# lxjeffffff/PagedAttention-Based-Transformer-Decoder-Inference-Framework

Hardware: AMD Instinct MI355X
Metric: decode tokens/sec at batch=64 seq_len=8192; % HBM-roofline (1/2/4/8 GPU) (higher is better)
Workload: dtype int8 GEMM (i32 acc) + fp16 KV attention (fp32 acc); 1 GPU; C3: INT8 decoder (MFMA i8 matmuls + fp16 paged attention), 24-layer/16-head/d=128, batch 64, KV context 8192, page 16; strong scaling: 64 rows over 1 GPU(s); global_batch=64, batch_per_gpu=64, seq_len=8192, page_size=16, parallelism=single GPU (no collective)

## Files before the change

pagedattention-based-transformer-decoder-inference-framework_amd/csrc/gemm_impl.hpp:

```cpp
#pragma once

#include "common.hpp"
#include "fp8.hpp"
#include "gemm.hpp"
#include "ln_wave.hpp"

namespace llm {

struct KvAppend {
  const int32_t* pos;
  const int32_t* page_table;
  const int32_t* rows;
  _Float16* k_pool;
  _Float16* v_pool;
  int num_beams, max_tiles, TS, num_pages, H, D;
  size_t page_stride;
  int fp8;
  float k_inv, v_inv;
};

struct GemmArgs {
  const uint8_t* A;
  int lda;
  int a_packed;
  const uint8_t* B;
  int M, N, K, KS;
  const float* sa;
  const float* sw;
  const float* bias;
  int act;
  float* C;
  int32_t* acc_out;
  int c_cols;
  int c_ld;
  _Float16* c16;
  KvAppend kv;
  unsigned long long* stamps;
  const float* ln_x;
  const _Float16* ln_emb;
  const int32_t* ln_tok;
  int ln_V;
  const float* ln_g;
  const float* ln_b;
  float ln_eps;
  uint8_t* act_out;
  float* sa_out;
  int partial;
  int w_keep;
  int xcd_map;
  unsigned* seam;
  int seam_n;
  int qdiag;
  int ksplit2;
};

__host__ __device__ constexpr int ln_row_stride(int K, int esize) { return K * esize + 32; }

__device__ __forceinline__ unsigned long long phase_clock() {
  unsigned long long t;
  asm volatile("s_memrealtime %0\n\ts_waitcnt lgkmcnt(0)" : "=s"(t)::"memory");
  return t;
}


template <int MT, int WAVES, int NT = 1>
constexpr int gemm_unroll() {
  return (MT >= 4 ? 2 : 4) * (WAVES == 4 ? 2 : 1) / (NT >= 4 ? 2 : 1);
}

__device__ __forceinline__ float apply_act(float y, int act) {
  if (act == LLM_ACT_RELU) return fmaxf(y, 0.f);
  if (act == LLM_ACT_GELU) return 0.5f * y * (1.f + erff(y * 0.70710678118654752f));
  return y;
}

enum class GemmKind { I8, F16 };

template <GemmKind KIND>
struct GemmTraits;
template <>
struct GemmTraits<GemmKind::I8> {
  static constexpr int KSTEP = 64, ESIZE = 1;
  using acc_t = i32x4;
  using elem_t = int32_t;
};
template <>
struct GemmTraits<GemmKind::F16> {
  static constexpr int KSTEP = 32, ESIZE = 2;
  using acc_t = f32x4;
  using elem_t = float;
};

template <GemmKind KIND, int ROWS, int WAVES>
__device__ __forceinline__ void ln_prologue(const GemmArgs& a, int m0, uint8_t* alds,
                                            float* sa_lds) {
  constexpr int ESIZE = GemmTraits<KIND>::ESIZE;
  constexpr int CPL = 8;
  const int lane = lane_id();
  const int w = wave_id_uniform();
  const int K = a.K;
  const int K4 = K >> 2;
  const int stride = ln_row_stride(K, ESIZE);
  const bool do_ln = a.ln_g != nullptr;
  LnRow<CPL> gm, bt;
  ln_wave_load(a.ln_g, K4, do_ln, gm);
  ln_wave_load(a.ln_b, K4, do_ln, bt);
  for (int r0 = w; r0 < ROWS; r0 += 2 * WAVES) {
    LnRow<CPL> x[2];
#pragma unroll
    for (int q = 0; q < 2; ++q) {
      const int r = r0 + q * WAVES;
      const int m = m0 + r;
      const bool ok = r < ROWS && m < a.M;
      if (a.ln_emb)
        ln_wave_load_f16(ok ? ln_embed_row(a.ln_emb, a.ln_tok, m, a.ln_V, K) : a.ln_emb, K4, ok,
                         x[q]);
      else
        ln_wave_load(a.ln_x + (size_t)m * K, K4, ok, x[q]);
    }
#pragma unroll
    for (int q = 0; q < 2; ++q) {
      const int r = r0 + q * WAVES;
      if (r >= ROWS) break;
      const bool mok = m0 + r < a.M;
      float am;
      if (do_ln) {
        am = ln_wave_compute(x[q], gm, bt, K, a.ln_eps);
      } else {
        am = 0.f;
#pragma unroll
        for (int j = 0; j < CPL; ++j)
#pragma unroll
          for (int e = 0; e < 4; ++e) am = fmaxf(am, fabsf(x[q].v[j][e]));
        am = ln_wave_max(am);
      }
      uint8_t* rowp = alds + (size_t)r * stride;
      if constexpr (KIND == GemmKind::I8) {
        const float scale = 127.f / (am + 1e-6f);
#pragma unroll
        for (int j = 0; j < CPL; ++j) {
          const int c = 64 * j + lane;
          if (c < K4)
            *reinterpret_cast<uint32_t*>(rowp + 4 * c) = mok ? ln_quant4(x[q].v[j], scale) : 0u;
        }
        if (lane == 0) sa_lds[r] = mok ? 1.0f / scale : 0.f;
      } else {
#pragma unroll
        for (int j = 0; j < CPL; ++j) {
          const int c = 64 * j + lane;
          if (c < K4)
            *reinterpret_cast<ln_f16x4*>(rowp + 8 * c) =
                mok ? ln_half4(x[q].v[j]) : ln_f16x4{0, 0, 0, 0};
        }
      }
    }
  }
}

__device__ __forceinline__ void seam_wait(unsigned* ctr, int n) {
  if (threadIdx.x == 0) {
    unsigned spins = 0;
    while (__hip_atomic_load(&ctr[0], __ATOMIC_RELAXED, __HIP_MEMORY_SCOPE_AGENT) < (unsigned)n) {
      __builtin_amdgcn_s_sleep(8);
      if (++spins > (1u << 21)) {
        __hip_atomic_store(&ctr[2], 1u, __ATOMIC_RELAXED, __HIP_MEMORY_SCOPE_AGENT);
        break;
      }
    }
    __builtin_amdgcn_fence(__ATOMIC_ACQUIRE, "agent");
  }
  __syncthreads();
}

template <GemmKind KIND, int MT, int NT, int WAVES, int DIAG = 0, int PRO = 0, int SEAM = 0>
__device__ __forceinline__ void gemm_tile(const GemmArgs& a, int bx, int by, int bz, int nz,
                                          int gx) {
  using Tr = GemmTraits<KIND>;
  using acc_t = typename Tr::acc_t;
  constexpr int KSTEP = Tr::KSTEP;
  constexpr int kUnroll = gemm_unroll<MT, WAVES, NT>();
  using elem_t = typename Tr::elem_t;
  using RedT = elem_t[MT * NT][4][64];
  extern __shared__ __attribute__((aligned(16))) uint8_t gemm_smem[];
  RedT* red;
  if constexpr (PRO == 0) {
    __shared__ elem_t red_static[WAVES][MT * NT][4][64];
    red = red_static;
  } else {
    red = reinterpret_cast<RedT*>(gemm_smem);
  }
  constexpr int ROWS_ = 16 * MT;
  const int a_stride = ln_row_stride(a.K, Tr::ESIZE);
  uint8_t* alds = gemm_smem;
  float* sa_lds = reinterpret_cast<float*>(gemm_smem + (size_t)ROWS_ * a_stride);

  const int lane = lane_id();
  const int w = wave_id_uniform();
  const int nt0 = bx * NT;
  const int m0 = by * 16 * MT;
  unsigned long long* stamp =
      a.stamps ? a.stamps + ((size_t)by * gx + bx) * 48 : nullptr;
  if (stamp && lane == 0) stamp[w] = phase_clock();
  const int wr = (w + bx) % WAVES;
  const int kz0 = (int)((bz * a.KS) / nz);
  const int kzn = (int)(((bz + 1) * a.KS) / nz) - kz0;
  const int ks0 = kz0 + (wr * kzn) / WAVES;
  const int ks1 = kz0 + ((wr + 1) * kzn) / WAVES;
  const int ntiles = (a.N + 15) >> 4;

  const int arow_lane = lane & 15;
  const int kgrp = lane >> 4;
  const bool apk = a.a_packed;
  const uint32_t a_bytes = apk ? (uint32_t)(((a.M + 15) / 16) * a.KS * 1024u)
                               : (uint32_t)((size_t)a.M * a.lda * Tr::ESIZE);
  const auto arsrc = __builtin_amdgcn_make_buffer_rsrc((void*)a.A, (short)0, a_bytes, 0x00020000);
  const uint32_t a_kstride = apk ? 1024u : (uint32_t)(KSTEP * Tr::ESIZE);
  const uint32_t a_kgrp_off = apk ? 0u : (uint32_t)(kgrp * (KSTEP / 4) * Tr::ESIZE);
  uint32_t a_row_off[MT];
#pragma unroll
  for (int mt = 0; mt < MT; ++mt) {
    const int row = m0 + mt * 16 + arow_lane;
    a_row_off[mt] = row >= a.M ? 0xFFFFFFF0u
                    : apk ? (uint32_t)((((m0 >> 4) + mt) * a.KS) * 1024u + lane * 16)
                          : (uint32_t)((size_t)row * a.lda * Tr::ESIZE);
  }
  const uint8_t* bbase = a.B + (size_t)nt0 * a.KS * 1024;
  const uint32_t b_bytes = (uint32_t)(min(NT, ntiles - nt0) * a.KS * 1024u);
  uint32_t b_lane_off[NT];
#pragma unroll
  for (int j = 0; j < NT; ++j) b_lane_off[j] = (uint32_t)j * a.KS * 1024u + lane * 16;
  const auto brsrc = __builtin_amdgcn_make_buffer_rsrc((void*)bbase, (short)0, b_bytes, 0x00020000);

  acc_t acc[MT][NT];
#pragma unroll
  for (int mt = 0; mt < MT; ++mt)
#pragma unroll
    for (int j = 0; j < NT; ++j) acc[mt][j] = acc_t{0, 0, 0, 0};

  struct Batch {
    u32x4 b[kUnroll][NT];
    u32x4 af[kUnroll][MT];
  };
  auto issue = [&](Batch& bt, int ks, bool do_a = true, bool do_b = true) {
#pragma unroll
    for (int u = 0; u < kUnroll; ++u) {
      const int kk = ks + u;
      const bool ok = kk < ks1;
#pragma unroll
      for (int j = 0; j < NT; ++j) {
        if (!do_b) break;
        const uint32_t boff = ok ? b_lane_off[j] + (uint32_t)kk * 1024u : 0xFFFFFFF0u;
        bt.b[u][j] = a.w_keep ? __builtin_amdgcn_raw_buffer_load_b128(brsrc, boff, 0, 0)
                              : __builtin_amdgcn_raw_buffer_load_b128(brsrc, boff, 0, 2);
      }
#pragma unroll
      for (int mt = 0; mt < MT; ++mt) {
        if (!do_a) break;
        if constexpr (PRO != 0) {
          const int r = mt * 16 + arow_lane;
          bt.af[u][mt] = ok ? *reinterpret_cast<const u32x4*>(alds + (size_t)r * a_stride +
                                                             16 * (4 * kk + kgrp))
                            : u32x4{0u, 0u, 0u, 0u};
          continue;
        }
        const uint32_t koff = (uint32_t)kk * a_kstride + a_kgrp_off;
        const uint32_t aoff = (ok && a_row_off[mt] != 0xFFFFFFF0u) ? a_row_off[mt] + koff : 0xFFFFFFF0u;
        if constexpr ((DIAG & 1) != 0)
          bt.af[u][mt] = u32x4{aoff, 0u, 0u, 0u};
        else
          bt.af[u][mt] = __builtin_amdgcn_raw_buffer_load_b128(arsrc, aoff, 0, 0);
      }
    }
  };
  auto compute = [&](const Batch& bt) {
#pragma unroll
    for (int u = 0; u < kUnroll; ++u) {
#pragma unroll
      for (int mt = 0; mt < MT; ++mt) {
        if constexpr (KIND == GemmKind::I8) {
#pragma unroll
          for (int j = 0; j < NT; ++j)
            acc[mt][j] = __builtin_amdgcn_mfma_i32_16x16x64_i8(
                __builtin_bit_cast(i32x4, bt.af[u][mt]), __builtin_bit_cast(i32x4, bt.b[u][j]),
                acc[mt][j], 0, 0, 0);
        } else if constexpr (KIND == GemmKind::F16) {
#pragma unroll
          for (int j = 0; j < NT; ++j)
            acc[mt][j] = __builtin_amdgcn_mfma_f32_16x16x32_f16(
                __builtin_bit_cast(f16x8, bt.af[u][mt]), __builtin_bit_cast(f16x8, bt.b[u][j]),
                acc[mt][j], 0, 0, 0);
        }
      }
    }
  };

  constexpr int ROWS = 16 * MT, COLS = 16 * NT, NTHR = WAVES * 64;
  constexpr int EPT = (ROWS * COLS + NTHR - 1) / NTHR;
  const KvAppend& kv = a.kv;
  const int hid = kv.H * kv.D;
  float e_scale[EPT], e_bias[EPT];
  int e_pos[EPT], e_br[EPT], e_page[EPT];
#pragma unroll
  for (int e = 0; e < EPT; ++e) {
    const int o = threadIdx.x + e * NTHR;
    const int m = m0 + o / COLS;
    const int n = nt0 * 16 + o % COLS;
    const bool valid = o < ROWS * COLS && m < a.M && n < a.N;
    e_scale[e] = 1.f;
    if constexpr (KIND == GemmKind::I8) {
      if (!PRO && valid && a.sa) e_scale[e] *= a.sa[m];
      if (valid && a.sw) e_scale[e] *= a.sw[n];
    }
    e_bias[e] = valid && a.bias && (!a.ksplit2 || bz == 0) ? a.bias[n] : 0.f;
    const bool kvcol = valid && kv.k_pool && n >= hid;
    e_pos[e] = kvcol ? kv.pos[m] : -1;
    e_br[e] = kvcol ? (kv.rows ? kv.rows[m] : m) : -1;
  }

  Batch b0, b1;
  bool b1_pre = false;
  if constexpr (PRO != 0) {
    bool pre = true;
#if LLM_TUNING
    pre = (a.qdiag & 2) == 0;
#endif
    if (pre && ks0 < ks1) issue(b0, ks0, false, true);
    if (pre && ks0 + kUnroll < ks1) {
      issue(b1, ks0 + kUnroll, false, true);
      b1_pre = true;
    }
    if constexpr (SEAM != 0) seam_wait(a.seam, a.seam_n);
#if LLM_TUNING
    if ((a.qdiag & 1) == 0)
#endif
    ln_prologue<KIND, ROWS_, WAVES>(a, m0, alds, sa_lds);
    __syncthreads();
    if constexpr (KIND == GemmKind::I8) {
#pragma unroll
      for (int e = 0; e < EPT; ++e) {
        const int o = threadIdx.x + e * NTHR;
        if (o < ROWS * COLS) e_scale[e] *= sa_lds[o / COLS];
      }
    }
    if (a.act_out && bx == 0) {
      const int KS = a.KS;
      for (int i = threadIdx.x; i < ROWS_ * KS * 4; i += NTHR) {
        const int r = i / (KS * 4), g = i % (KS * 4);
        const int m = m0 + r;
        if (m >= a.M) continue;
        const size_t off = ((size_t)((m >> 4) * KS + (g >> 2)) * 64 + (m & 15) + 16 * (g & 3)) * 16;
        *reinterpret_cast<u32x4*>(a.act_out + off) =
            *reinterpret_cast<const u32x4*>(alds + (size_t)r * a_stride + 16 * g);
      }
      if (KIND == GemmKind::I8 && a.sa_out && threadIdx.x < ROWS_ && m0 + (int)threadIdx.x < a.M)
        a.sa_out[m0 + threadIdx.x] = sa_lds[threadIdx.x];
    }
  }

  {
    int ks = ks0;
    bool b0_b = PRO == 0;
#if LLM_TUNING
    if constexpr (PRO != 0) b0_b = (a.qdiag & 2) != 0;
#endif
    if (ks < ks1) issue(b0, ks, true, b0_b);
#pragma unroll
    for (int e = 0; e < EPT; ++e) {
      const int o = threadIdx.x + e * NTHR;
      const int n = nt0 * 16 + o % COLS;
      const int p = e_pos[e], br = e_br[e];
      int page = -1;
      if (p >= 0 && br >= 0 && br < kv.num_beams && p / kv.TS < kv.max_tiles) {
        const int which = n >= 2 * hid;
        const int h = (n - hid * (1 + which)) / kv.D;
        page = kv.page_table[((size_t)br * kv.H + h) * kv.max_tiles + p / kv.TS];
        if (page >= kv.num_pages) page = -1;
      }
      e_page[e] = page;
    }
    while (ks < ks1) {
      if (ks + kUnroll < ks1) {
        issue(b1, ks + kUnroll, true, !b1_pre);
        b1_pre = false;
      }
      compute(b0);
      ks += kUnroll;
      if (ks >= ks1) break;
      if (ks + kUnroll < ks1) issue(b0, ks + kUnroll);
      compute(b1);
      ks += kUnroll;
    }
  }

  if (stamp && lane == 0) stamp[16 + w] = phase_clock();
  if constexpr ((DIAG & 2) != 0) {
    int32_t x = 0;
#pragma unroll
    for (int mt = 0; mt < MT; ++mt)
#pragma unroll
      for (int j = 0; j < NT; ++j) x ^= (int32_t)acc[mt][j][0] ^ (int32_t)acc[mt][j][3];
    if (lane == 0 && a.C) a.C[bx] = (float)x;
    if (stamp && lane == 0) stamp[32 + w] = phase_clock();
    return;
  }
  if constexpr (PRO != 0) __syncthreads();
#pragma unroll
  for (int mt = 0; mt < MT; ++mt)
#pragma unroll
    for (int j = 0; j < NT; ++j)
#pragma unroll
      for (int r = 0; r < 4; ++r) red[wr][mt * NT + j][r][lane] = acc[mt][j][r];
  __syncthreads();

#pragma unroll
  for (int e = 0; e < EPT; ++e) {
#pragma clang fp contract(off)
    const int o = threadIdx.x + e * NTHR;
    if (o >= ROWS * COLS) break;
    const int cl = o % COLS;
    const int row = o / COLS;
    const int j = cl >> 4;
    const int col = cl & 15;
    const int mt = row >> 4;
    const int rl = row & 15;
    const int src_lane = (rl >> 2) * 16 + col;
    const int reg = rl & 3;
    const int m = m0 + row;
    const int n = (nt0 + j) * 16 + col;
    if (m >= a.M || n >= a.N) continue;
    float y;
    if constexpr (KIND == GemmKind::I8) {
      int32_t s = 0;
#pragma unroll
      for (int ww = 0; ww < WAVES; ++ww) s += red[ww][mt * NT + j][reg][src_lane];
#if LLM_TUNING
      if (a.partial) {
        a.acc_out[((size_t)bz * a.M + m) * a.N + n] = s;
        continue;
      }
#endif
      if (a.acc_out) a.acc_out[(size_t)m * a.N + n] = s;
      y = (float)s * e_scale[e];
      if (a.bias) y = y + e_bias[e];
      if (a.ksplit2) {
        atomicAdd(a.C + (size_t)m * a.c_ld + n, y);
        continue;
      }
    } else {
      float s = 0.f;
#pragma unroll
      for (int ww = 0; ww < WAVES; ++ww) s += red[ww][mt * NT + j][reg][src_lane];
      y = a.bias ? s + e_bias[e] : s;
    }
    y = apply_act(y, a.act);
    if (a.C && n < a.c_cols) a.C[(size_t)m * a.c_ld + n] = y;
    if (a.c16) a.c16[a_frag_off_f16(m, n, a.N >> 5)] = (_Float16)y;
    if (e_page[e] >= 0) {
      const int which = n >= 2 * hid;
      const int i = n - hid * (1 + which);
      const int d = i % kv.D;
      const int p = e_pos[e];
      const size_t off = (size_t)e_page[e] * kv.page_stride + (size_t)(p % kv.TS) * kv.D + d;
      if (kv.fp8)
        reinterpret_cast<uint8_t*>(which ? kv.v_pool : kv.k_pool)[off] =
            (uint8_t)fp8_e4m3_byte(y, which ? kv.v_inv : kv.k_inv);
      else
        (which ? kv.v_pool : kv.k_pool)[off] = (_Float16)y;
    }
  }
  if (stamp && lane == 0) stamp[32 + w] = phase_clock();
}

template <GemmKind KIND, int MT, int NT, int WAVES, int DIAG = 0, int PRO = 0>
__global__ __launch_bounds__(WAVES * 64) void gemm_kernel(GemmArgs a) {
  int bx = blockIdx.x, by = blockIdx.y, bz = blockIdx.z;
#if LLM_TUNING
  if (a.xcd_map) {
    const int per = 8 / (int)gridDim.z;
    const int lin = blockIdx.x + gridDim.x * (blockIdx.y + gridDim.y * blockIdx.z);
    const int xcd = lin & 7;
    const int tile = (lin >> 3) * per + xcd % per;
    bz = xcd / per;
    bx = tile % (int)gridDim.x;
    by = tile / (int)gridDim.x;
  }
#endif
  gemm_tile<KIND, MT, NT, WAVES, DIAG, PRO>(a, bx, by, bz, (int)gridDim.z, (int)gridDim.x);
}

template <typename T, int EPL>
__global__ void pack_kernel(const T* __restrict__ W, T* __restrict__ P, int K, int N, int KS,
                            int ntiles) {
  const size_t idx = (size_t)blockIdx.x * blockDim.x + threadIdx.x;
  const size_t total = (size_t)ntiles * KS * 64;
  if (idx >= total) return;
  const int lane = idx & 63;
  const size_t blk = idx >> 6;
  const int ks = blk % KS;
  const int nt = blk / KS;
  const int n = nt * 16 + (lane & 15);
  const int kb = ks * (4 * EPL) + (lane >> 4) * EPL;
  T* dst = P + idx * EPL;
#pragma unroll
  for (int j = 0; j < EPL; ++j) {
    const int k = kb + j;
    dst[j] = (k < K && n < N) ? W[(size_t)k * N + n] : T(0);
  }
}

namespace {

inline int pick_nt(int N, int M) {
  if (M <= 16) return 1;
  const int ntiles = (N + 15) / 16;
  const int mblocks = (M + 63) / 64;
  return (ntiles % 2 == 0 && (ntiles / 2) * mblocks >= 192) ? 2 : 1;
}

template <GemmKind KIND, int MT, int NT, int WAVES>
size_t ln_lds_bytes(int K) {
  const size_t img = (size_t)16 * MT * ln_row_stride(K, GemmTraits<KIND>::ESIZE) + 16 * MT * 4;
  const size_t red = (size_t)WAVES * MT * NT * 4 * 64 * 4;
  return img > red ? img : red;
}
constexpr size_t kLnLdsMax = 160 * 1024;

struct GemmForm {
  int mt;
  int nt;
  int waves;
  int kslices;
  int prologue;
};

template <GemmKind KIND, int MT, int NT>
hipError_t launch_gemm_nt(const GemmArgs& a, const GemmForm& f, int mblocks, hipStream_t st) {
  const int ntiles = (a.N + 15) / 16;
  const dim3 grid((ntiles + NT - 1) / NT, mblocks, f.kslices);
  if constexpr (NT <= 2) {
    if (f.prologue) {
      const size_t lds = ln_lds_bytes<KIND, MT, NT, 8>(a.K);
      hipLaunchKernelGGL((gemm_kernel<KIND, MT, NT, 8, 0, 1>), grid, dim3(512), lds, st, a);
      return hipGetLastError();
    }
  }
  if constexpr (MT * NT * 8 <= 64) {
    if (f.waves == 8) {
      hipLaunchKernelGGL((gemm_kernel<KIND, MT, NT, 8>), grid, dim3(512), 0, st, a);
      return hipGetLastError();
    }
  }
  hipLaunchKernelGGL((gemm_kernel<KIND, MT, NT, 4>), grid, dim3(256), 0, st, a);
  return hipGetLastError();
}

template <GemmKind KIND, int MT>
hipError_t launch_gemm_mt(const GemmArgs& a, const GemmForm& f, int mblocks, hipStream_t st) {
#if LLM_TUNING
  if (f.nt == 4) return launch_gemm_nt<KIND, MT, 4>(a, f, mblocks, st);
  if (f.nt == 3) return launch_gemm_nt<KIND, MT, 3>(a, f, mblocks, st);
#endif
  return f.nt == 2 ? launch_gemm_nt<KIND, MT, 2>(a, f, mblocks, st)
                   : launch_gemm_nt<KIND, MT, 1>(a, f, mblocks, st);
}

}

namespace {

inline int pick_waves(const GemmArgs&, int) { return 8; }

struct TileChoice {
  int nt, waves, mrows;
};
inline bool narrow_tile_for(int M, int N, int K, TileChoice& t) {
  if (M <= 16 || M > 64) return false;
  const int ntiles = (N + 15) / 16;
  if (M > 32) {
    if (ntiles >= 256) return false;
    t = TileChoice{2, 8, 16};
    return true;
  }
  if (ntiles < 384) {
    t = K >= 4096 ? TileChoice{1, 8, 16} : TileChoice{1, 4, 16};
    return true;
  }
  if (ntiles < 512) {
    t = TileChoice{1, 4, 16};
    return true;
  }
  return false;
}
inline bool narrow_decode_tile(const GemmArgs& a, int kstep, TileChoice& t) {
  if ((a.ln_x && a.ln_g) || a.partial) return false;
  if (a.ksplit2 && a.M > 32 && a.M <= 64) {
    t = TileChoice{2, 8, 64};
    return true;
  }
  return narrow_tile_for(a.M, a.N, a.KS * kstep, t);
}

inline GemmForm gemm_form(const GemmArgs& a, int kstep, int nt_override = 0,
                          int waves_override = 0, int mrows_override = 0, int ks_override = 0) {
  TileChoice tc{0, 0, 0};
  const bool narrow = nt_override == 0 && waves_override == 0 && mrows_override == 0 &&
                      narrow_decode_tile(a, kstep, tc);
  if (narrow) {
    nt_override = tc.nt;
    waves_override = tc.waves;
    mrows_override = tc.mrows;
  }
  const int NT = nt_override > 0 ? nt_override : pick_nt(a.N, a.M);
  const int waves = waves_override > 0 ? waves_override : pick_waves(a, NT);
  int mrows = a.M <= 16 ? 16 : a.M <= 32 ? 32 : 64;
  if (mrows == 64 && NT == 1 && (a.N + 15) / 16 < 256 && !a.ln_x && !a.partial) mrows = 32;
  if (mrows_override > 0) mrows = mrows_override;
  GemmForm f{};
  f.mt = mrows == 16 ? 1 : mrows == 32 ? 2 : 4;
  f.nt = NT == 2 ? 2 : 1;
#if LLM_TUNING
  if ((NT == 3 || NT == 4) && !a.ln_x) f.nt = NT;
#endif
  f.prologue = a.ln_x != nullptr;
  f.waves = f.prologue || (f.mt * f.nt * 8 <= 64 && waves != 4) ? 8 : 4;
  f.kslices = a.partial ? std::max(1, ks_override) : a.ksplit2 ? 2 : 1;
  return f;
}

template <GemmKind KIND>
hipError_t launch_gemm(const GemmArgs& a_in, hipStream_t st, int nt_override = 0,
                       int waves_override = 0, int mrows_override = 0, int ks_override = 0) {
  GemmArgs a = a_in;
  const GemmForm f = gemm_form(a, GemmTraits<KIND>::KSTEP, nt_override, waves_override,
                               mrows_override, ks_override);
  const int mblocks = (a.M + 16 * f.mt - 1) / (16 * f.mt);
  const int tiles = ((a.N + 15) / 16 + f.nt - 1) / f.nt * mblocks;
  if (a.xcd_map && (f.kslices < 2 || 8 % f.kslices != 0 || (tiles * f.kslices) % 8 != 0))
    a.xcd_map = 0;
  if (f.mt == 1) return launch_gemm_mt<KIND, 1>(a, f, mblocks, st);
  if (f.mt == 2) return launch_gemm_mt<KIND, 2>(a, f, mblocks, st);
  return launch_gemm_mt<KIND, 4>(a, f, mblocks, st);
}

}
}
```

pagedattention-based-transformer-decoder-inference-framework_amd/csrc/tune/gemm_tune.hip:

```cpp
#include "gemm_impl.hpp"

using namespace llm;

__global__ void gemm_end_stamp_kernel(unsigned long long* t) {
  if (threadIdx.x == 0) *t = phase_clock();
}

extern "C" int i8_gemm_stamps(int nt, int waves, int mrows, const int8_t* A, const void* W_packed,
                              float* C, int M, int N, int K, const float* sa, const float* sw,
                              unsigned long long* stamps, unsigned long long* end_stamp,
                              void* stream) {
  GemmArgs a{};
  a.a_packed = 1;
  a.A = reinterpret_cast<const uint8_t*>(A);
  a.lda = K;
  a.B = static_cast<const uint8_t*>(W_packed);
  a.M = M; a.N = N; a.K = K; a.KS = K / 64;
  a.sa = sa; a.sw = sw; a.C = C; a.c_cols = N; a.c_ld = N;
  a.stamps = stamps;
  hipStream_t st = as_stream(stream);
  hipError_t e = hipSuccess;
  const int ntiles = N / 16;
  const int diag = waves >> 8;
  if (diag == 0) {
    e = launch_gemm<GemmKind::I8>(a, st, nt, waves, mrows);
  } else {
    LLM_REQUIRE((nt == 2 && mrows == 64) || (nt == 1 && mrows == 32), "i8_gemm_stamps: diag shape");
    auto go = [&](auto kern, int NTv, int mr) {
      hipLaunchKernelGGL(kern, dim3((ntiles + NTv - 1) / NTv, (M + mr - 1) / mr), dim3(512), 0, st, a);
    };
    if (nt == 2) {
      if (diag == 1) go(gemm_kernel<GemmKind::I8, 4, 2, 8, 1>, 2, 64);
      else if (diag == 2) go(gemm_kernel<GemmKind::I8, 4, 2, 8, 2>, 2, 64);
      else go(gemm_kernel<GemmKind::I8, 4, 2, 8, 3>, 2, 64);
    } else {
      if (diag == 1) go(gemm_kernel<GemmKind::I8, 2, 1, 8, 1>, 1, 32);
      else if (diag == 2) go(gemm_kernel<GemmKind::I8, 2, 1, 8, 2>, 1, 32);
      else go(gemm_kernel<GemmKind::I8, 2, 1, 8, 3>, 1, 32);
    }
    e = hipGetLastError();
  }
  if (e == hipSuccess) {
    hipLaunchKernelGGL(gemm_end_stamp_kernel, dim3(1), dim3(64), 0, st, end_stamp);
    e = hipGetLastError();
  }
  return e == hipSuccess ? LLM_OK : fail(LLM_ERR_HIP, "i8_gemm_stamps");
}

extern "C" int i8_gemm_tune(int nt, int waves, int mrows, int a_packed, const int8_t* A, int lda,
                            const void* W_packed, float* C, int M, int N, int K, const float* sa,
                            const float* sw, void* stream) {
  GemmArgs a{};
  a.a_packed = a_packed;
  a.A = reinterpret_cast<const uint8_t*>(A);
  a.lda = lda;
  a.B = static_cast<const uint8_t*>(W_packed);
  a.M = M; a.N = N; a.K = K; a.KS = K / 64;
  a.sa = sa; a.sw = sw; a.C = C; a.c_cols = N; a.c_ld = N;
  hipError_t e = launch_gemm<GemmKind::I8>(a, as_stream(stream), nt, waves, mrows);
  return e == hipSuccess ? LLM_OK : fail(LLM_ERR_HIP, "i8_gemm_tune");
}

extern "C" int i8_gemm_tune_qpro(const float* x, const void* W_packed, float* C, int M, int N,
                                 int K, const float* sw, int qdiag, void* stream) {
  LLM_REQUIRE(quant_prologue_ok(M, N, K), "i8_gemm_tune_qpro: shape");
  GemmArgs a{};
  a.a_packed = 1;
  a.B = static_cast<const uint8_t*>(W_packed);
  a.M = M; a.N = N; a.K = K; a.KS = K / 64;
  a.sw = sw; a.C = C; a.c_cols = N; a.c_ld = N;
  a.ln_x = x;
  a.ln_eps = 1e-5f;
  a.qdiag = qdiag;
  hipError_t e = launch_gemm<GemmKind::I8>(a, as_stream(stream));
  return e == hipSuccess ? LLM_OK : fail(LLM_ERR_HIP, "i8_gemm_tune_qpro");
}

extern "C" int i8_gemm_tune_sk(int nt, int waves, int mrows, int kslices, int xcd_map,
                               const int8_t* A, const void* W_packed, int32_t* acc_out, int M,
                               int N, int K, void* stream) {
  LLM_REQUIRE(kslices >= 1 && kslices <= 8 && K % 64 == 0 && N % 16 == 0, "i8_gemm_tune_sk: shape");
  GemmArgs a{};
  a.a_packed = 1;
  a.A = reinterpret_cast<const uint8_t*>(A);
  a.lda = K;
  a.B = static_cast<const uint8_t*>(W_packed);
  a.M = M; a.N = N; a.K = K; a.KS = K / 64;
  a.partial = 1;
  a.acc_out = acc_out;
  a.xcd_map = xcd_map;
  hipError_t e = launch_gemm<GemmKind::I8>(a, as_stream(stream), nt, waves, mrows, kslices);
  return e == hipSuccess ? LLM_OK : fail(LLM_ERR_HIP, "i8_gemm_tune_sk");
}

__global__ __launch_bounds__(512) void gemm_pair_f16_kernel(GemmArgs a1, GemmArgs a2, int n1,
                                                            unsigned* sync) {
  const int wg = blockIdx.x;
  if (wg < n1) {
    gemm_tile<GemmKind::F16, 1, 1, 8, 0, 0>(a1, wg, 0, 0, 1, n1);
    __syncthreads();
    if (threadIdx.x == 0) {
      __builtin_amdgcn_fence(__ATOMIC_RELEASE, "agent");
      __hip_atomic_fetch_add(&sync[0], 1u, __ATOMIC_RELAXED, __HIP_MEMORY_SCOPE_AGENT);
    }
  }
  gemm_tile<GemmKind::F16, 1, 1, 8, 0, 1, 1>(a2, wg, 0, 0, 1, (int)gridDim.x);
  if (threadIdx.x == 0) {
    const unsigned old = __hip_atomic_fetch_add(&sync[1], 1u, __ATOMIC_RELAXED, __HIP_MEMORY_SCOPE_AGENT);
    if (old == gridDim.x - 1) {
      __hip_atomic_store(&sync[0], 0u, __ATOMIC_RELAXED, __HIP_MEMORY_SCOPE_AGENT);
      __hip_atomic_store(&sync[1], 0u, __ATOMIC_RELAXED, __HIP_MEMORY_SCOPE_AGENT);
    }
  }
}

extern "C" int f16_gemm_pair_tune(const void* A1, const void* W1, float* x, const float* ln_g,
                                  const float* ln_b, const void* W2, const float* b2, void* C16,
                                  int M, int K, int N1, int N2, unsigned* sync, int fused,
                                  void* stream) {
  LLM_REQUIRE(M >= 1 && M <= 16 && K == N1 && K % 32 == 0 && N1 % 16 == 0 && N2 % 32 == 0 &&
                  ln_fusable(LLM_F16, M, K) && N2 / 16 >= N1 / 16 && N2 / 16 <= 256,
              "f16_gemm_pair_tune: shape");
  GemmArgs a1{};
  a1.a_packed = 1;
  a1.A = static_cast<const uint8_t*>(A1);
  a1.B = static_cast<const uint8_t*>(W1);
  a1.M = M; a1.N = N1; a1.K = K; a1.KS = K / 32;
  a1.C = x; a1.c_cols = N1; a1.c_ld = N1;
  a1.w_keep = 1;
  GemmArgs a2{};
  a2.a_packed = 1;
  a2.B = static_cast<const uint8_t*>(W2);
  a2.M = M; a2.N = N2; a2.K = N1; a2.KS = N1 / 32;
  a2.bias = b2; a2.act = LLM_ACT_RELU;
  a2.c16 = static_cast<_Float16*>(C16);
  a2.c_cols = 0; a2.c_ld = N2;
  a2.ln_x = x; a2.ln_g = ln_g; a2.ln_b = ln_b; a2.ln_eps = 1e-5f;
  a2.w_keep = 1;
  a2.seam = sync;
  a2.seam_n = N1 / 16;
  hipStream_t st = as_stream(stream);
  hipError_t e;
  if (!fused) {
    e = launch_gemm<GemmKind::F16>(a1, st);
    if (e == hipSuccess) e = launch_gemm<GemmKind::F16>(a2, st);
  } else {
    const size_t lds = ln_lds_bytes<GemmKind::F16, 1, 1, 8>(N1);
    hipLaunchKernelGGL(gemm_pair_f16_kernel, dim3(N2 / 16), dim3(512), lds, st, a1, a2, N1 / 16,
                       sync);
    e = hipGetLastError();
  }
  return e == hipSuccess ? LLM_OK : fail(LLM_ERR_HIP, "f16_gemm_pair_tune");
}

extern "C" int f16_gemm_tune(int nt, int waves, int mrows, int a_packed, const void* A, int lda,
                             const void* W_packed, float* C, int M, int N, int K, void* stream) {
  GemmArgs a{};
  a.a_packed = a_packed;
  a.A = static_cast<const uint8_t*>(A);
  a.lda = lda;
  a.B = static_cast<const uint8_t*>(W_packed);
  a.M = M; a.N = N; a.K = K; a.KS = K / 32;
  a.C = C; a.c_cols = N; a.c_ld = N;
  hipError_t e = launch_gemm<GemmKind::F16>(a, as_stream(stream), nt, waves, mrows);
  return e == hipSuccess ? LLM_OK : fail(LLM_ERR_HIP, "f16_gemm_tune");
}

struct WeightGemmTuneArgs {
  int dtype;
  const void* A;
  int lda, a_packed;
  const void* W_packed;
  int M, N, K;
  const float* sa;
  const float* sw;
  const float* bias;
  int act;
  float* C;
  int c_cols, c_ld;
  void* C16;
  const float* ln_x;
  const void* ln_emb;
  const int32_t* ln_tok;
  int ln_V;
  const float* ln_g;
  const float* ln_b;
  float ln_eps;
  void* act_out;
  float* sa_out;
  int w_keep, ln_quant_only, ksplit2;
  int has_kv;
  const int32_t* kv_pos;
  const int32_t* kv_page_table;
  const int32_t* kv_rows;
  void* kv_k_pool;
  void* kv_v_pool;
  int kv_num_beams, kv_max_tiles, kv_page_size, kv_num_pages, kv_H, kv_D;
  long long kv_page_stride;
  int kv_dtype;
  float kv_k_inv_scale, kv_v_inv_scale;
};

extern "C" int weight_gemm_tune(const WeightGemmTuneArgs* t, void* stream) {
  LLM_REQUIRE(t, "weight_gemm_tune: NULL arguments");
  KvAppendView kv;
  kv.pos = t->kv_pos;
  kv.page_table = t->kv_page_table;
  kv.rows = t->kv_rows;
  kv.k_pool = t->kv_k_pool;
  kv.v_pool = t->kv_v_pool;
  kv.num_beams = t->kv_num_beams; kv.max_tiles = t->kv_max_tiles;
  kv.page_size = t->kv_page_size; kv.num_pages = t->kv_num_pages;
  kv.H = t->kv_H; kv.D = t->kv_D;
  kv.page_stride = (size_t)t->kv_page_stride;
  kv.kv_dtype = t->kv_dtype;
  kv.k_inv_scale = t->kv_k_inv_scale; kv.v_inv_scale = t->kv_v_inv_scale;
  WeightGemm g;
  g.dtype = t->dtype;
  g.A = t->A; g.lda = t->lda; g.a_packed = t->a_packed;
  g.W_packed = t->W_packed;
  g.M = t->M; g.N = t->N; g.K = t->K;
  g.sa = t->sa; g.sw = t->sw; g.bias = t->bias; g.act = t->act;
  g.C = t->C; g.c_cols = t->c_cols; g.c_ld = t->c_ld;
  g.C16 = t->C16;
  g.kv = t->has_kv ? &kv : nullptr;
  g.ln_x = t->ln_x;
  g.ln_emb = static_cast<const _Float16*>(t->ln_emb);
  g.ln_tok = t->ln_tok; g.ln_V = t->ln_V;
  g.ln_g = t->ln_g; g.ln_b = t->ln_b; g.ln_eps = t->ln_eps;
  g.act_out = t->act_out; g.sa_out = t->sa_out;
  g.w_keep = t->w_keep;
  g.ln_quant_only = t->ln_quant_only;
  g.ksplit2 = t->ksplit2;
  return weight_gemm(g, as_stream(stream));
}

extern "C" int gemm_ln_fusable_tune(int dtype, int M, int K) { return ln_fusable(dtype, M, K); }

extern "C" int gemm_quant_prologue_ok_tune(int M, int N, int K) {
  return quant_prologue_ok(M, N, K);
}

extern "C" int gemm_form_tune(int dtype, int M, int N, int K, int prologue, int ksplit2, int nt,
                              int waves, int mrows, int* form) {
  LLM_REQUIRE(form && M > 0 && N > 0 && K > 0 && (dtype == LLM_I8 || dtype == LLM_F16) &&
                  prologue >= 0 && prologue <= 2,
              "gemm_form_tune: bad arguments");
  const int kstep = dtype == LLM_I8 ? 64 : 32;
  static const float never_read = 0.f;
  GemmArgs a{};
  a.M = M; a.N = N; a.K = K; a.KS = K / kstep;
  a.ln_x = prologue ? &never_read : nullptr;
  a.ln_g = prologue == 1 ? &never_read : nullptr;
  a.ksplit2 = ksplit2;
  const GemmForm f = gemm_form(a, kstep, nt, waves, mrows);
  form[0] = f.mt; form[1] = f.nt; form[2] = f.waves; form[3] = f.kslices; form[4] = f.prologue;
  return LLM_OK;
}
```

Baseline: 3791 tokens/s.

## Stage epilogue operands in LDS per wave and vectorize GEMM epilogue stores

Replaces the per-thread, per-element gathering of scales, bias, KV positions and page-table entries with a per-block record in LDS. Each of four waves loads one operand kind before the main loop, and the page-table lookups are computed once per row and head slot. The epilogue now has each thread process four adjacent columns, using vector reads from the reduction buffer and vector stores for C, the fp16 output and the fp8/fp16 KV pool writes. It also restructures the b1 prefetch issue in the main loop, adds an NT=8 prologue variant under tuning, and lowers the LDS cap, which adds dynamic LDS use to every launch and may reduce occupancy.

```diff
diff --git a/pagedattention-based-transformer-decoder-inference-framework_amd/csrc/gemm_impl.hpp b/pagedattention-based-transformer-decoder-inference-framework_amd/csrc/gemm_impl.hpp
--- a/pagedattention-based-transformer-decoder-inference-framework_amd/csrc/gemm_impl.hpp
+++ b/pagedattention-based-transformer-decoder-inference-framework_amd/csrc/gemm_impl.hpp
@@ -56,6 +56,20 @@
 
 __host__ __device__ constexpr int ln_row_stride(int K, int esize) { return K * esize + 32; }
 
+__host__ __device__ constexpr size_t pro_union_bytes(int rows, int K, int esize, int waves,
+                                                     int tiles) {
+  const size_t img = (size_t)rows * ln_row_stride(K, esize) + (size_t)rows * 4;
+  const size_t red = (size_t)waves * tiles * 1024;
+  return ((img > red ? img : red) + 15) & ~(size_t)15;
+}
+
+__host__ __device__ constexpr int kv_slots_max(int cols, int D) {
+  return D <= 0 ? 0 : (cols - 2) / D + 2 < cols ? (cols - 2) / D + 2 : cols;
+}
+__host__ __device__ constexpr size_t epi_rec_bytes(int rows, int cols, int kv_D) {
+  return (size_t)(2 * rows + 2 * cols + rows * kv_slots_max(cols, kv_D)) * 4;
+}
+
 __device__ __forceinline__ unsigned long long phase_clock() {
   unsigned long long t;
   asm volatile("s_memrealtime %0\n\ts_waitcnt lgkmcnt(0)" : "=s"(t)::"memory");
@@ -295,27 +309,88 @@
   };
 
   constexpr int ROWS = 16 * MT, COLS = 16 * NT, NTHR = WAVES * 64;
-  constexpr int EPT = (ROWS * COLS + NTHR - 1) / NTHR;
+  constexpr int CL = (COLS + 63) / 64;
+  static_assert(WAVES >= 4 && ROWS <= 64, "epilogue record: one wave per operand kind");
   const KvAppend& kv = a.kv;
+  const bool has_kv = kv.k_pool != nullptr;
   const int hid = kv.H * kv.D;
-  float e_scale[EPT], e_bias[EPT];
-  int e_pos[EPT], e_br[EPT], e_page[EPT];
-#pragma unroll
-  for (int e = 0; e < EPT; ++e) {
-    const int o = threadIdx.x + e * NTHR;
-    const int m = m0 + o / COLS;
-    const int n = nt0 * 16 + o % COLS;
-    const bool valid = o < ROWS * COLS && m < a.M && n < a.N;
-    e_scale[e] = 1.f;
-    if constexpr (KIND == GemmKind::I8) {
-      if (!PRO && valid && a.sa) e_scale[e] *= a.sa[m];
-      if (valid && a.sw) e_scale[e] *= a.sw[n];
-    }
-    e_bias[e] = valid && a.bias && (!a.ksplit2 || bz == 0) ? a.bias[n] : 0.f;
-    const bool kvcol = valid && kv.k_pool && n >= hid;
-    e_pos[e] = kvcol ? kv.pos[m] : -1;
-    e_br[e] = kvcol ? (kv.rows ? kv.rows[m] : m) : -1;
-  }
+  size_t rec_off = 0;
+  if constexpr (PRO != 0) rec_off = pro_union_bytes(ROWS, a.K, Tr::ESIZE, WAVES, MT * NT);
+  float* r_sa = reinterpret_cast<float*>(gemm_smem + rec_off);
+  int* r_pos = reinterpret_cast<int*>(r_sa + ROWS);
+  float* r_sw = r_sa + 2 * ROWS;
+  float* r_bias = r_sw + COLS;
+  int* r_page = reinterpret_cast<int*>(r_bias + COLS);
+  int kv_g0 = 0, kv_ns = 0;
+  if (has_kv) {
+    const int nlo = max(nt0 * 16, hid), nhi = min(nt0 * 16 + COLS, a.N);
+    if (nlo < nhi) {
+      kv_g0 = (nlo - hid) / kv.D;
+      kv_ns = min((nhi - 1 - hid) / kv.D - kv_g0 + 1, kv_slots_max(COLS, kv.D));
+    }
+  }
+  float e_sa = 1.f, e_sw[CL], e_bias[CL];
+#pragma unroll
+  for (int i = 0; i < CL; ++i) e_sw[i] = 1.f, e_bias[i] = 0.f;
+  int e_pos = -1, e_br = -1, e_tile = 0, e_page[2] = {-1, -1};
+  if (w == 0 && kv_ns > 0 && lane < ROWS && m0 + lane < a.M) {
+    e_pos = kv.pos[m0 + lane];
+    e_br = kv.rows ? kv.rows[m0 + lane] : m0 + lane;
+  }
+  auto load_page = [&](int s) {
+    const int g = kv_g0 + s;
+    const int h = g >= kv.H ? g - kv.H : g;
+    return kv.page_table[((size_t)e_br * kv.H + h) * kv.max_tiles + e_tile];
+  };
+  auto load_operands = [&]() {
+    if (w == 0) {
+      if (e_pos >= 0) e_tile = e_pos / kv.TS;
+      if (!(e_pos >= 0 && e_br >= 0 && e_br < kv.num_beams && e_tile < kv.max_tiles)) e_pos = -1;
+#pragma unroll
+      for (int s = 0; s < 2; ++s)
+        if (e_pos >= 0 && s < kv_ns) e_page[s] = load_page(s);
+    } else if (w == 1) {
+      if constexpr (KIND == GemmKind::I8) {
+        if constexpr (PRO == 0)
+          if (a.sa && lane < ROWS && m0 + lane < a.M) e_sa = a.sa[m0 + lane];
+      }
+    } else if (w == 2) {
+      if constexpr (KIND == GemmKind::I8) {
+#pragma unroll
+        for (int i = 0; i < CL; ++i) {
+          const int c = lane + 64 * i, n = nt0 * 16 + c;
+          if (a.sw && c < COLS && n < a.N) e_sw[i] = a.sw[n];
+        }
+      }
+    } else if (w == 3) {
+#pragma unroll
+      for (int i = 0; i < CL; ++i) {
+        const int c = lane + 64 * i, n = nt0 * 16 + c;
+        if (a.bias && (!a.ksplit2 || bz == 0) && c < COLS && n < a.N) e_bias[i] = a.bias[n];
+      }
+    }
+  };
+  auto store_operands = [&]() {
+    if (w == 0) {
+      if (has_kv && lane < ROWS) {
+        r_pos[lane] = e_pos;
+        for (int s = 0; s < kv_ns; ++s) {
+          const int page = e_pos < 0 ? -1 : s < 2 ? e_page[s] : load_page(s);
+          r_page[s * ROWS + lane] = page < kv.num_pages ? page : -1;
+        }
+      }
+    } else if (w == 1) {
+      if (lane < ROWS) r_sa[lane] = e_sa;
+    } else if (w == 2) {
+#pragma unroll
+      for (int i = 0; i < CL; ++i)
+        if (lane + 64 * i < COLS) r_sw[lane + 64 * i] = e_sw[i];
+    } else if (w == 3) {
+#pragma unroll
+      for (int i = 0; i < CL; ++i)
+        if (lane + 64 * i < COLS) r_bias[lane + 64 * i] = e_bias[i];
+    }
+  };
 
   Batch b0, b1;
   bool b1_pre = false;
@@ -329,6 +404,7 @@
       issue(b1, ks0 + kUnroll, false, true);
       b1_pre = true;
     }
+    load_operands();
     if constexpr (SEAM != 0) seam_wait(a.seam, a.seam_n);
 #if LLM_TUNING
     if ((a.qdiag & 1) == 0)
@@ -336,11 +412,7 @@
     ln_prologue<KIND, ROWS_, WAVES>(a, m0, alds, sa_lds);
     __syncthreads();
     if constexpr (KIND == GemmKind::I8) {
-#pragma unroll
-      for (int e = 0; e < EPT; ++e) {
-        const int o = threadIdx.x + e * NTHR;
-        if (o < ROWS * COLS) e_scale[e] *= sa_lds[o / COLS];
-      }
+      if (w == 1 && lane < ROWS && m0 + lane < a.M) e_sa = sa_lds[lane];
     }
     if (a.act_out && bx == 0) {
       const int KS = a.KS;
@@ -364,31 +436,16 @@
     if constexpr (PRO != 0) b0_b = (a.qdiag & 2) != 0;
 #endif
     if (ks < ks1) issue(b0, ks, true, b0_b);
-#pragma unroll
-    for (int e = 0; e < EPT; ++e) {
-      const int o = threadIdx.x + e * NTHR;
-      const int n = nt0 * 16 + o % COLS;
-      const int p = e_pos[e], br = e_br[e];
-      int page = -1;
-      if (p >= 0 && br >= 0 && br < kv.num_beams && p / kv.TS < kv.max_tiles) {
-        const int which = n >= 2 * hid;
-        const int h = (n - hid * (1 + which)) / kv.D;
-        page = kv.page_table[((size_t)br * kv.H + h) * kv.max_tiles + p / kv.TS];
-        if (page >= kv.num_pages) page = -1;
-      }
-      e_page[e] = page;
-    }
+    if (ks + kUnroll < ks1) issue(b1, ks + kUnroll, true, !b1_pre);
+    if constexpr (PRO == 0) load_operands();
     while (ks < ks1) {
-      if (ks + kUnroll < ks1) {
-        issue(b1, ks + kUnroll, true, !b1_pre);
-        b1_pre = false;
-      }
       compute(b0);
       ks += kUnroll;
       if (ks >= ks1) break;
       if (ks + kUnroll < ks1) issue(b0, ks + kUnroll);
       compute(b1);
       ks += kUnroll;
+      if (ks + kUnroll < ks1) issue(b1, ks + kUnroll);
     }
   }
 
@@ -410,62 +467,131 @@
     for (int j = 0; j < NT; ++j)
 #pragma unroll
       for (int r = 0; r < 4; ++r) red[wr][mt * NT + j][r][lane] = acc[mt][j][r];
+  store_operands();
   __syncthreads();
 
-#pragma unroll
-  for (int e = 0; e < EPT; ++e) {
+  const int c4 = threadIdx.x & 3;
+  const int qs = (threadIdx.x >> 2) & 15;
+  const int rl = ((qs >> 1) & 3) * 4 + (qs & 1) + 2 * (qs >> 3);
+  const int red_reg = rl & 3, red_lane = (rl >> 2) * 16 + 4 * c4;
+  auto aligned = [](const void* p, unsigned n) { return (reinterpret_cast<uintptr_t>(p) & (n - 1)) == 0; };
+  const bool c_vec = ((a.c_cols | a.c_ld) & 3) == 0 && aligned(a.C, 16);
+  const bool acc_vec = aligned(a.acc_out, 16);
+  const bool c16_vec = aligned(a.c16, 8);
+  const bool kv_vec = has_kv && ((kv.D | (int)(kv.page_stride & 3)) & 3) == 0 &&
+                      aligned(kv.k_pool, 8) && aligned(kv.v_pool, 8);
+  for (int t = w; t < MT * NT; t += WAVES) {
 #pragma clang fp contract(off)
-    const int o = threadIdx.x + e * NTHR;
-    if (o >= ROWS * COLS) break;
-    const int cl = o % COLS;
-    const int row = o / COLS;
-    const int j = cl >> 4;
-    const int col = cl & 15;
-    const int mt = row >> 4;
-    const int rl = row & 15;
-    const int src_lane = (rl >> 2) * 16 + col;
-    const int reg = rl & 3;
+    const int mt = t / NT, j = t % NT;
+    const int row = mt * 16 + rl;
+    const int cl = j * 16 + 4 * c4;
     const int m = m0 + row;
-    const int n = (nt0 + j) * 16 + col;
+    const int n = nt0 * 16 + cl;
     if (m >= a.M || n >= a.N) continue;
-    float y;
+    const f32x4 bias4 = *reinterpret_cast<const f32x4*>(r_bias + cl);
+    float y[4];
     if constexpr (KIND == GemmKind::I8) {
-      int32_t s = 0;
-#pragma unroll
-      for (int ww = 0; ww < WAVES; ++ww) s += red[ww][mt * NT + j][reg][src_lane];
+      i32x4 s = {0, 0, 0, 0};
+#pragma unroll
+      for (int ww = 0; ww < WAVES; ++ww)
+        s += *reinterpret_cast<const i32x4*>(&red[ww][t][red_reg][red_lane]);
+      int32_t* acc_dst = nullptr;
 #if LLM_TUNING
-      if (a.partial) {
-        a.acc_out[((size_t)bz * a.M + m) * a.N + n] = s;
+      if (a.partial) acc_dst = a.acc_out + ((size_t)bz * a.M + m) * a.N + n;
+      else
+#endif
+      if (a.acc_out) acc_dst = a.acc_out + (size_t)m * a.N + n;
+      if (acc_dst) {
+        if (acc_vec) {
+          *reinterpret_cast<i32x4*>(acc_dst) = s;
+        } else {
+#pragma unroll
+          for (int i = 0; i < 4; ++i) acc_dst[i] = s[i];
+        }
+      }
+#if LLM_TUNING
+      if (a.partial) continue;
+#endif
+      const float sa_row = r_sa[row];
+      const f32x4 sw4 = *reinterpret_cast<const f32x4*>(r_sw + cl);
+#pragma unroll
+      for (int i = 0; i < 4; ++i) {
+        y[i] = (float)s[i] * (sa_row * sw4[i]);
+        if (a.bias) y[i] = y[i] + bias4[i];
+      }
+      if (a.ksplit2) {
+#pragma unroll
+        for (int i = 0; i < 4; ++i) atomicAdd(a.C + (size_t)m * a.c_ld + n + i, y[i]);
         continue;
       }
-#endif
-      if (a.acc_out) a.acc_out[(size_t)m * a.N + n] = s;
-      y = (float)s * e_scale[e];
-      if (a.bias) y = y + e_bias[e];
-      if (a.ksplit2) {
-        atomicAdd(a.C + (size_t)m * a.c_ld + n, y);
-        continue;
-      }
     } else {
-      float s = 0.f;
-#pragma unroll
-      for (int ww = 0; ww < WAVES; ++ww) s += red[ww][mt * NT + j][reg][src_lane];
-      y = a.bias ? s + e_bias[e] : s;
-    }
-    y = apply_act(y, a.act);
-    if (a.C && n < a.c_cols) a.C[(size_t)m * a.c_ld + n] = y;
-    if (a.c16) a.c16[a_frag_off_f16(m, n, a.N >> 5)] = (_Float16)y;
-    if (e_page[e] >= 0) {
-      const int which = n >= 2 * hid;
-      const int i = n - hid * (1 + which);
-      const int d = i % kv.D;
-      const int p = e_pos[e];
-      const size_t off = (size_t)e_page[e] * kv.page_stride + (size_t)(p % kv.TS) * kv.D + d;
-      if (kv.fp8)
-        reinterpret_cast<uint8_t*>(which ? kv.v_pool : kv.k_pool)[off] =
-            (uint8_t)fp8_e4m3_byte(y, which ? kv.v_inv : kv.k_inv);
-      else
-        (which ? kv.v_pool : kv.k_pool)[off] = (_Float16)y;
+      f32x4 s = {0.f, 0.f, 0.f, 0.f};
+#pragma unroll
+      for (int ww = 0; ww < WAVES; ++ww)
+        s += *reinterpret_cast<const f32x4*>(&red[ww][t][red_reg][red_lane]);
+#pragma unroll
+      for (int i = 0; i < 4; ++i) y[i] = a.bias ? s[i] + bias4[i] : s[i];
+    }
+#pragma unroll
+    for (int i = 0; i < 4; ++i) y[i] = apply_act(y[i], a.act);
+    if (a.C) {
+      float* dst = a.C + (size_t)m * a.c_ld + n;
+      if (c_vec && n + 3 < a.c_cols) {
+        *reinterpret_cast<f32x4*>(dst) = f32x4{y[0], y[1], y[2], y[3]};
+      } else {
+#pragma unroll
+        for (int i = 0; i < 4; ++i)
+          if (n + i < a.c_cols) dst[i] = y[i];
+      }
+    }
+    if (a.c16) {
+      _Float16* dst = a.c16 + a_frag_off_f16(m, n, a.N >> 5);
+      if (c16_vec) {
+        *reinterpret_cast<ln_f16x4*>(dst) =
+            ln_f16x4{(_Float16)y[0], (_Float16)y[1], (_Float16)y[2], (_Float16)y[3]};
+      } else {
+#pragma unroll
+        for (int i = 0; i < 4; ++i) dst[i] = (_Float16)y[i];
+      }
+    }
+    if (has_kv && n >= hid) {
+      const int p = r_pos[row];
+      if (p < 0) continue;
+      auto kv_dst = [&](int nn, bool& is_v, size_t& off) {
+        const int g = (nn - hid) / kv.D;
+        const int slot = g - kv_g0;
+        if (slot >= kv_ns) return false;
+        const int page = r_page[slot * ROWS + row];
+        if (page < 0) return false;
+        is_v = g >= kv.H;
+        off = (size_t)page * kv.page_stride + (size_t)(p % kv.TS) * kv.D + (nn - hid - g * kv.D);
+        return true;
+      };
+      bool is_v;
+      size_t off;
+      if (kv_vec) {
+        if (!kv_dst(n, is_v, off)) continue;
+        if (kv.fp8) {
+          const float inv = is_v ? kv.v_inv : kv.k_inv;
+          *reinterpret_cast<uint32_t*>(reinterpret_cast<uint8_t*>(is_v ? kv.v_pool : kv.k_pool) +
+                                       off) =
+              fp8_e4m3_byte(y[0], inv) | fp8_e4m3_byte(y[1], inv) << 8 |
+              fp8_e4m3_byte(y[2], inv) << 16 | fp8_e4m3_byte(y[3], inv) << 24;
+        } else {
+          *reinterpret_cast<ln_f16x4*>((is_v ? kv.v_pool : kv.k_pool) + off) =
+              ln_f16x4{(_Float16)y[0], (_Float16)y[1], (_Float16)y[2], (_Float16)y[3]};
+        }
+      } else {
+#pragma unroll
+        for (int i = 0; i < 4; ++i) {
+          if (!kv_dst(n + i, is_v, off)) continue;
+          if (kv.fp8)
+            reinterpret_cast<uint8_t*>(is_v ? kv.v_pool : kv.k_pool)[off] =
+                (uint8_t)fp8_e4m3_byte(y[i], is_v ? kv.v_inv : kv.k_inv);
+          else
+            (is_v ? kv.v_pool : kv.k_pool)[off] = (_Float16)y[i];
+        }
+      }
     }
   }
   if (stamp && lane == 0) stamp[32 + w] = phase_clock();
@@ -518,12 +644,11 @@
 }
 
 template <GemmKind KIND, int MT, int NT, int WAVES>
-size_t ln_lds_bytes(int K) {
-  const size_t img = (size_t)16 * MT * ln_row_stride(K, GemmTraits<KIND>::ESIZE) + 16 * MT * 4;
-  const size_t red = (size_t)WAVES * MT * NT * 4 * 64 * 4;
-  return img > red ? img : red;
-}
-constexpr size_t kLnLdsMax = 160 * 1024;
+size_t gemm_lds_bytes(const GemmArgs& a, bool prologue) {
+  const size_t rec = epi_rec_bytes(16 * MT, 16 * NT, a.kv.k_pool ? a.kv.D : 0);
+  return rec + (prologue ? pro_union_bytes(16 * MT, a.K, GemmTraits<KIND>::ESIZE, WAVES, MT * NT) : 0);
+}
+constexpr size_t kLnLdsMax = 140 * 1024;
 
 struct GemmForm {
   int mt;
@@ -537,26 +662,30 @@
 hipError_t launch_gemm_nt(const GemmArgs& a, const GemmForm& f, int mblocks, hipStream_t st) {
   const int ntiles = (a.N + 15) / 16;
   const dim3 grid((ntiles + NT - 1) / NT, mblocks, f.kslices);
-  if constexpr (NT <= 2) {
+  if constexpr (NT <= 2 || (LLM_TUNING && KIND == GemmKind::I8 && MT == 1)) {
     if (f.prologue) {
-      const size_t lds = ln_lds_bytes<KIND, MT, NT, 8>(a.K);
+      const size_t lds = gemm_lds_bytes<KIND, MT, NT, 8>(a, true);
       hipLaunchKernelGGL((gemm_kernel<KIND, MT, NT, 8, 0, 1>), grid, dim3(512), lds, st, a);
       return hipGetLastError();
     }
   }
   if constexpr (MT * NT * 8 <= 64) {
     if (f.waves == 8) {
-      hipLaunchKernelGGL((gemm_kernel<KIND, MT, NT, 8>), grid, dim3(512), 0, st, a);
+      const size_t lds = gemm_lds_bytes<KIND, MT, NT, 8>(a, false);
+      hipLaunchKernelGGL((gemm_kernel<KIND, MT, NT, 8>), grid, dim3(512), lds, st, a);
       return hipGetLastError();
     }
   }
-  hipLaunchKernelGGL((gemm_kernel<KIND, MT, NT, 4>), grid, dim3(256), 0, st, a);
+  const size_t lds = gemm_lds_bytes<KIND, MT, NT, 4>(a, false);
+  hipLaunchKernelGGL((gemm_kernel<KIND, MT, NT, 4>), grid, dim3(256), lds, st, a);
   return hipGetLastError();
 }
 
 template <GemmKind KIND, int MT>
 hipError_t launch_gemm_mt(const GemmArgs& a, const GemmForm& f, int mblocks, hipStream_t st) {
 #if LLM_TUNING
+  if constexpr (KIND == GemmKind::I8 && MT == 1)
+    if (f.nt == 8) return launch_gemm_nt<KIND, MT, 8>(a, f, mblocks, st);
   if (f.nt == 4) return launch_gemm_nt<KIND, MT, 4>(a, f, mblocks, st);
   if (f.nt == 3) return launch_gemm_nt<KIND, MT, 3>(a, f, mblocks, st);
 #endif
@@ -620,6 +749,7 @@
   f.nt = NT == 2 ? 2 : 1;
 #if LLM_TUNING
   if ((NT == 3 || NT == 4) && !a.ln_x) f.nt = NT;
+  if ((NT == 4 || NT == 8) && a.ln_x && !a.ln_g && f.mt == 1 && kstep == 64) f.nt = NT;
 #endif
   f.prologue = a.ln_x != nullptr;
   f.waves = f.prologue || (f.mt * f.nt * 8 <= 64 && waves != 4) ? 8 : 4;
diff --git a/pagedattention-based-transformer-decoder-inference-framework_amd/csrc/tune/gemm_tune.hip b/pagedattention-based-transformer-decoder-inference-framework_amd/csrc/tune/gemm_tune.hip
--- a/pagedattention-based-transformer-decoder-inference-framework_amd/csrc/tune/gemm_tune.hip
+++ b/pagedattention-based-transformer-decoder-inference-framework_amd/csrc/tune/gemm_tune.hip
@@ -27,7 +27,8 @@
   } else {
     LLM_REQUIRE((nt == 2 && mrows == 64) || (nt == 1 && mrows == 32), "i8_gemm_stamps: diag shape");
     auto go = [&](auto kern, int NTv, int mr) {
-      hipLaunchKernelGGL(kern, dim3((ntiles + NTv - 1) / NTv, (M + mr - 1) / mr), dim3(512), 0, st, a);
+      hipLaunchKernelGGL(kern, dim3((ntiles + NTv - 1) / NTv, (M + mr - 1) / mr), dim3(512),
+                         epi_rec_bytes(mr, 16 * NTv, 0), st, a);
     };
     if (nt == 2) {
       if (diag == 1) go(gemm_kernel<GemmKind::I8, 4, 2, 8, 1>, 2, 64);
@@ -71,8 +72,11 @@
   a.sw = sw; a.C = C; a.c_cols = N; a.c_ld = N;
   a.ln_x = x;
   a.ln_eps = 1e-5f;
-  a.qdiag = qdiag;
-  hipError_t e = launch_gemm<GemmKind::I8>(a, as_stream(stream));
+  a.qdiag = qdiag & 3;
+  const int nt = qdiag >> 8;
+  LLM_REQUIRE(nt == 0 || nt == 1 || nt == 2 || nt == 4 || nt == 8, "i8_gemm_tune_qpro: column tiles");
+  hipError_t e = nt ? launch_gemm<GemmKind::I8>(a, as_stream(stream), nt, 8, 16)
+                    : launch_gemm<GemmKind::I8>(a, as_stream(stream));
   return e == hipSuccess ? LLM_OK : fail(LLM_ERR_HIP, "i8_gemm_tune_qpro");
 }
 
@@ -145,7 +149,7 @@
     e = launch_gemm<GemmKind::F16>(a1, st);
     if (e == hipSuccess) e = launch_gemm<GemmKind::F16>(a2, st);
   } else {
-    const size_t lds = ln_lds_bytes<GemmKind::F16, 1, 1, 8>(N1);
+    const size_t lds = gemm_lds_bytes<GemmKind::F16, 1, 1, 8>(a2, true);
     hipLaunchKernelGGL(gemm_pair_f16_kernel, dim3(N2 / 16), dim3(512), lds, st, a1, a2, N1 / 16,
                        sync);
     e = hipGetLastError();
```

Measured after the change: 3816 tokens/s (median of 6 runs). No clear change (+0.7%).
